# fevzibabaoglu/adaptive-edge-aware-jpeg

Measured on AMD Instinct MI355X. Metric: megapixels/sec encode (Canny+quadtree+DCT+quant), 4K batch, higher is better.
Workload: dtype f32

## Files before the change

adaptive_edge_aware_jpeg_amd/csrc/canny.hip:

```cpp
#include "aej_common.h"
#include "aej_launch.h"
#include <stdlib.h>

namespace aej {

__device__ __forceinline__ int reflect101(int i, int n)
{
    if (n == 1) return 0;
    while (i < 0 || i >= n) {
        if (i < 0) i = -i;
        if (i >= n) i = 2 * (n - 1) - i;
    }
    return i;
}

__device__ __forceinline__ int cdiv(int a, int b) { return (a + b - 1) / b; }

__device__ __forceinline__ long long xcd_remap(long long id, long long n)
{
    const long long q = n / 8, r = n % 8, xcd = id % 8, k = id / 8;
    return (xcd < r ? xcd * (q + 1) : r * (q + 1) + (xcd - r) * q) + k;
}

__device__ __forceinline__ bool locate_tile(const Geom &g, int TW, int TH, int t, int &layer, int &tx, int &ty, int &ntx, int &nty, int &tbase)
{
    tbase = 0;
    for (int l = 0; l < g.nl; l++) {
        ntx = cdiv(g.w[l], TW); nty = cdiv(g.h[l], TH);
        int n = ntx * nty;
        if (t < n) { layer = l; ty = t / ntx; tx = t - ty * ntx; return true; }
        t -= n; tbase += n;
    }
    return false;
}

static long long tiles_per_image(const Geom &g, int TW, int TH)
{
    long long n = 0;
    for (int l = 0; l < g.nl; l++) n += (long long)((g.w[l] + TW - 1) / TW) * ((g.h[l] + TH - 1) / TH);
    return n;
}
long long hyst_tiles_per_image(const Geom &g) { return tiles_per_image(g, kHystTile, kHystTile); }
int hyst_ring_slots(const Geom &g)
{
    const long long t2 = 2 * hyst_tiles_per_image(g) * g.B;
    int p = 1;
    while (2LL * p <= t2) p *= 2;
    return p;
}

__global__ __launch_bounds__(256) void k_clahe_pad_hist(Geom g, const unsigned char *__restrict__ u8, int *__restrict__ tile_hist)
{
    const int l = blockIdx.y, b = blockIdx.z;
    const int w = g.w[l], h = g.h[l];
    if ((w % 4) == 0 && (h % 4) == 0) return;
    const int wp = g.ctw[l] * 4, hp = g.cth[l] * 4;
    const int nright = (wp - w) * hp;
    const int nbottom = w * (hp - h);
    const unsigned char *src = u8 + (long long)b * g.pstride + g.poff[l];
    int *hist = tile_hist + ((long long)b * 3 + l) * 16 * 256;
    for (int i = blockIdx.x * 256 + threadIdx.x; i < nright + nbottom; i += gridDim.x * 256) {
        int x, y;
        if (i < nright) { y = i / (wp - w); x = w + (i - y * (wp - w)); }
        else { int k = i - nright; y = h + k / w; x = k % w; }
        int v = src[(long long)reflect101(y, h) * w + reflect101(x, w)];
        atomicAdd(&hist[((y / g.cth[l]) * 4 + (x / g.ctw[l])) * 256 + v], 1);
    }
}

__global__ __launch_bounds__(256) void k_clahe_lut(Geom g, const int *__restrict__ tile_hist, unsigned char *__restrict__ lut, double clip_limit)
{
    __shared__ int s[256];
    __shared__ int s_red[4];
    const int tile = blockIdx.x, l = blockIdx.y, b = blockIdx.z, tid = threadIdx.x;
    const long long base = (((long long)b * 3 + l) * 16 + tile) * 256;
    const int area = g.ctw[l] * g.cth[l];
    const float lutScale = 255.0f / (float)area;
    int clip = 0x7fffffff;
    if (clip_limit > 0.0) { clip = (int)(clip_limit * (double)area / 256.0); if (clip < 1) clip = 1; }
    int hv = tile_hist[base + tid];
    int excess = hv > clip ? hv - clip : 0;
    if (hv > clip) hv = clip;
    int v = excess;
    for (int o = 32; o > 0; o >>= 1) v += __shfl_down(v, o);
    if ((tid & 63) == 0) s_red[tid >> 6] = v;
    __syncthreads();
    const int clipped = s_red[0] + s_red[1] + s_red[2] + s_red[3];
    const int batch = clipped / 256;
    int resid = clipped - batch * 256;
    hv += batch;
    if (resid != 0) {
        int step = 256 / resid;
        if (step < 1) step = 1;
        if (tid % step == 0 && tid / step < resid) hv++;
    }
    s[tid] = hv;
    __syncthreads();
    for (int o = 1; o < 256; o <<= 1) {
        int t = tid >= o ? s[tid - o] : 0;
        __syncthreads();
        s[tid] += t;
        __syncthreads();
    }
    float f = (float)s[tid] * lutScale;
    int r = __float2int_rn(f);
    lut[base + tid] = (unsigned char)(r < 0 ? 0 : r > 255 ? 255 : r);
}

constexpr int kBT = 256;
constexpr int kBTW = 128, kBTH = 32;
constexpr int kBAW = kBTW + 8;
constexpr int kBAW4 = kBAW / 4;
constexpr int kBAH = kBTH + 6;
constexpr int kBGH = kBTH + 4;
constexpr int kBGW = kBAW + 4;
constexpr int kBGW2 = kBGW / 2;
static_assert(kBGW % 4 == 0, "Gaussian rows keep 8-byte alignment");
constexpr int kBStripMax = 15;
constexpr int kASlots = kBT / kBAW4;
constexpr int kAIter = (kBAH + kASlots - 1) / kASlots;
constexpr int kBRows = (kBGH + kASlots - 1) / kASlots;
static_assert(kASlots * kBRows >= kBGH && kASlots * kAIter >= kBAH, "thread -> row mapping must cover the tile");
constexpr float kTwo24 = 16777216.0f, kTwo22 = 4194304.0f;
constexpr int kHistCopies = 6;
constexpr int kHistStride = 257;

struct __attribute__((aligned(16))) BlurLds {
    int colq[kBAW];
    float colXa[kBAW], colXa1[kBAW];
    int colT1[kBAW], colT2[kBAW];
    int rowq[kBAH];
    float rowYa[kBAH], rowYa1[kBAH];
    int rowT1[kBAH], rowT2[kBAH];
    int cls[8];
    int pkey[2];
    float cw[3][512];
    unsigned int hist[kHistCopies * kHistStride];
    float4 P[2][256];
    unsigned int A[kBAH * kBAW4];
    unsigned int G[kBGH * kBGW2];
};
static_assert(3 * sizeof(BlurLds) <= 160 * 1024, "three workgroups per CU");

__device__ __forceinline__ int half_diff(unsigned a, int ah, unsigned b, int bh)
{
    int d;
    if (ah == 0 && bh == 0) asm("v_sub_u32_sdwa %0, %1, %2 dst_sel:DWORD dst_unused:UNUSED_PAD src0_sel:WORD_0 src1_sel:WORD_0" : "=v"(d) : "v"(b), "v"(a));
    else if (ah == 0)       asm("v_sub_u32_sdwa %0, %1, %2 dst_sel:DWORD dst_unused:UNUSED_PAD src0_sel:WORD_1 src1_sel:WORD_0" : "=v"(d) : "v"(b), "v"(a));
    else if (bh == 0)       asm("v_sub_u32_sdwa %0, %1, %2 dst_sel:DWORD dst_unused:UNUSED_PAD src0_sel:WORD_0 src1_sel:WORD_1" : "=v"(d) : "v"(b), "v"(a));
    else                    asm("v_sub_u32_sdwa %0, %1, %2 dst_sel:DWORD dst_unused:UNUSED_PAD src0_sel:WORD_1 src1_sel:WORD_1" : "=v"(d) : "v"(b), "v"(a));
    return d;
}

template <int T>
__device__ __forceinline__ float pair_w(const BlurLds &L, unsigned a, int ah, unsigned b, int bh)
{
    return *reinterpret_cast<const float *>(reinterpret_cast<const char *>(L.cw[T]) + 1024 + half_diff(a, ah, b, bh));
}

__device__ __forceinline__ float tap_fma(unsigned p, int h, float wgt, float sum)
{
    float r;
    if (h) asm("v_fma_mix_f32 %0, %1, %2, %3 op_sel:[1,0,0] op_sel_hi:[1,0,0]" : "=v"(r) : "v"(p), "v"(wgt), "v"(sum));
    else   asm("v_fma_mix_f32 %0, %1, %2, %3 op_sel_hi:[1,0,0]" : "=v"(r) : "v"(p), "v"(wgt), "v"(sum));
    return r;
}
__device__ __forceinline__ float tap_first(unsigned p, int h, float wgt)
{
    float r;
    if (h) asm("v_fma_mix_f32 %0, %1, %2, 0 op_sel:[1,0,0] op_sel_hi:[1,0,0]" : "=v"(r) : "v"(p), "v"(wgt));
    else   asm("v_fma_mix_f32 %0, %1, %2, 0 op_sel_hi:[1,0,0]" : "=v"(r) : "v"(p), "v"(wgt));
    return r;
}

__device__ __forceinline__ float clahe_blend(float l11, float l12, float l21, float l22, float xa, float xa1, float ya, float ya1)
{
    float pa = l11 * xa1, pb = l12 * xa, pc = l21 * xa1, pd = l22 * xa;
    float top = pa + pb, bot = pc + pd;
    float t1 = top * ya1, t2 = bot * ya;
    return t1 + t2;
}

__device__ __forceinline__ void blur_prefetch(const unsigned char *src, int w, int h, int x0, int y0, bool aligned, unsigned int (&raw)[kAIter])
{
    const int t = threadIdx.x;
    const int col = t % kBAW4, slot = t / kBAW4;
    if (slot >= kASlots) return;
#pragma unroll
    for (int k = 0; k < kAIter; k++) {
        const int j = slot + kASlots * k;
        if (j < kBAH) {
            if (aligned) {
                raw[k] = *reinterpret_cast<const unsigned int *>(src + (long long)(y0 - 3 + j) * w + (x0 - 4) + 4 * col);
            } else {
                const unsigned char *row = src + (long long)reflect101(y0 - 3 + j, h) * w;
                unsigned int v = 0;
#pragma unroll
                for (int q = 0; q < 4; q++) v |= (unsigned int)row[reflect101(x0 - 4 + 4 * col + q, w)] << (8 * q);
                raw[k] = v;
            }
        }
    }
}

__device__ __forceinline__ bool locate_blur_strip(const Geom &g, int strip, int t, int &layer, int &sx, int &ty)
{
    for (int l = 0; l < g.nl; l++) {
        int ntx = cdiv(g.w[l], kBTW), nty = cdiv(g.h[l], kBTH), nsx = cdiv(ntx, strip);
        int n = nsx * nty;
        if (t < n) { layer = l; ty = t / nsx; sx = t - ty * nsx; return true; }
        t -= n;
    }
    return false;
}


template <bool DUMP>
__global__ __launch_bounds__(kBT) __attribute__((amdgpu_waves_per_eu(3, 3))) void k_clahe_blur(Geom g, CannyBuffers cb, int strip)
{
    __shared__ BlurLds L;
    const int tid = threadIdx.x;
    const long long wg = xcd_remap(blockIdx.x, gridDim.x);
    const int strips = gridDim.x / g.B;
    const int b = (int)(wg / strips);
    int l, sx, ty;
    if (!locate_blur_strip(g, strip, (int)(wg - (long long)b * strips), l, sx, ty)) return;
    const int w = g.w[l], h = g.h[l];
    const int ntx = cdiv(w, kBTW);
    const int y0 = ty * kBTH;
    const int tx_begin = sx * strip, tx_end = min(ntx, tx_begin + strip);
    const long long pbase = (long long)b * g.pstride + g.poff[l];
    const unsigned char *src = cb.u8a + pbase;
    const unsigned char *glut = cb.lut + ((long long)b * 3 + l) * 4096;

    auto is_aligned = [&](int tx) {
        int x0 = tx * kBTW;
        return x0 >= 4 && y0 >= 3 && x0 + kBTW + 4 <= w && y0 + kBTH + 3 <= h && (w % 4) == 0;
    };
    unsigned int raw[kAIter];
    blur_prefetch(src, w, h, tx_begin * kBTW, y0, is_aligned(tx_begin), raw);

    static_assert(512 % kBT == 0, "weight table set-up assumes whole rounds");
#pragma unroll
    for (int i = tid; i < 512; i += kBT) {
        const int d = i - 256;
        const float cwv = i == 0 ? 0.f : cb.color_w[d < 0 ? -d : d];
        L.cw[0][i] = (cb.space_w[5] * cwv) * kTwo24;
        L.cw[1][i] = (cb.space_w[1] * cwv) * kTwo24;
        L.cw[2][i] = (cb.space_w[0] * cwv) * kTwo24;
    }
    for (int i = tid; i < kHistCopies * kHistStride; i += kBT) L.hist[i] = 0;
    if (tid < 2) L.pkey[tid] = -1;
    if (tid < kBAH) {
        const int j = tid;
        const int gy = reflect101(y0 - 3 + j, h);
        const float inv_th = 1.0f / (float)g.cth[l];
        float tyf = (float)gy * inv_th - 0.5f;
        int ty1 = (int)floorf(tyf), ty2 = ty1 + 1;
        float ya = tyf - (float)ty1;
        L.rowYa[j] = ya; L.rowYa1[j] = 1.0f - ya;
        if (ty1 < 0) ty1 = 0;
        if (ty2 > 3) ty2 = 3;
        L.rowT1[j] = ty1; L.rowT2[j] = ty2;
    }
    __syncthreads();
    {
        bool rchg = false;
        if (tid < kBAH) {
            const int j = tid;
            const int key = (L.rowT1[j] << 2) | L.rowT2[j], key0 = (L.rowT1[0] << 2) | L.rowT2[0];
            rchg = j > 0 && key != ((L.rowT1[j - 1] << 2) | L.rowT2[j - 1]);
            if (rchg) L.cls[3] = key;
            if (j == 0) L.cls[2] = key;
            L.rowq[j] = key != key0 ? (int)sizeof(L.P[0]) : 0;
        }
        const int n = __syncthreads_count(rchg);
        if (tid == 0) L.cls[5] = n;
    }
    unsigned char *dst = cb.u8b + pbase;

    for (int tx = tx_begin; tx < tx_end; tx++) {
        const int x0 = tx * kBTW;
        const bool full = x0 + kBTW <= w && y0 + kBTH <= h && (w % 4) == 0;
        if (tid == 0) L.cls[4] = 0;
        if (tid < kBAW) {
            const int gx = reflect101(x0 - 4 + tid, w);
            const float inv_tw = 1.0f / (float)g.ctw[l];
            float txf = (float)gx * inv_tw - 0.5f;
            int tx1 = (int)floorf(txf), tx2 = tx1 + 1;
            float xa = txf - (float)tx1;
            L.colXa[tid] = xa; L.colXa1[tid] = 1.0f - xa;
            if (tx1 < 0) tx1 = 0;
            if (tx2 > 3) tx2 = 3;
            L.colT1[tid] = tx1; L.colT2[tid] = tx2;
        }
        __syncthreads();
        if (tid < kBAW) {
            const int key = (L.colT1[tid] << 2) | L.colT2[tid], key0 = (L.colT1[0] << 2) | L.colT2[0];
            const bool chg = tid > 0 && key != ((L.colT1[tid - 1] << 2) | L.colT2[tid - 1]);
            if (chg) { atomicAdd(&L.cls[4], 1); L.cls[1] = key; }
            if (tid == 0) { L.cls[0] = key; }
            L.colq[tid] = key != key0 ? (int)sizeof(L.P[0]) : 0;
        }
        __syncthreads();
        const int nchg_c = L.cls[4], nchg_r = L.cls[5];
        const bool fast = nchg_c + nchg_r <= 1;
        if (fast) {
            const int key_s0 = (L.cls[0] << 4) | L.cls[2];
            const int key_s1 = (L.cls[nchg_c] << 4) | L.cls[2 + nchg_r];
            const bool need1 = nchg_c + nchg_r == 1;
            const bool build0 = L.pkey[0] != key_s0, build1 = need1 && L.pkey[1] != key_s1;
            if (build0 || build1) {
                for (int e = tid; e < 512; e += kBT) {
                    const int v = e & 255, slot = e >> 8;
                    const int key = slot ? key_s1 : key_s0;
                    if (slot ? build1 : build0) {
                        const int ckey = key >> 4, rkey = key & 15;
                        const int tx1 = ckey >> 2, tx2 = ckey & 3, ty1 = rkey >> 2, ty2 = rkey & 3;
                        L.P[slot][v] = make_float4((float)glut[(ty1 * 4 + tx1) * 256 + v], (float)glut[(ty1 * 4 + tx2) * 256 + v],
                                                   (float)glut[(ty2 * 4 + tx1) * 256 + v], (float)glut[(ty2 * 4 + tx2) * 256 + v]);
                    }
                }
                __syncthreads();
                if (tid < 2 && (tid ? build1 : build0)) L.pkey[tid] = tid ? key_s1 : key_s0;
            }
        }
        int tq = tid;
        asm volatile("" : "+v"(tq));
        const int acol = tq % kBAW4, aslot = tq / kBAW4;
        if (aslot < kASlots) {
            const float4 xa = reinterpret_cast<const float4 *>(L.colXa)[acol], xa1 = reinterpret_cast<const float4 *>(L.colXa1)[acol];
            if (fast) {
                const int4 cq = reinterpret_cast<const int4 *>(L.colq)[acol];
                const char *Pb = reinterpret_cast<const char *>(&L.P[0][0]);
#pragma unroll
                for (int k = 0; k < kAIter; k++) {
                    const int j = aslot + kASlots * k;
                    if (j < kBAH) {
                        const unsigned int rv = raw[k];
                        const int rq = L.rowq[j];
                        const float ya = L.rowYa[j], ya1 = L.rowYa1[j];
                        const float4 f0 = *reinterpret_cast<const float4 *>(Pb + ((rv & 0xffu) * 16u + (unsigned)(cq.x + rq)));
                        const float4 f1 = *reinterpret_cast<const float4 *>(Pb + (((rv >> 8) & 0xffu) * 16u + (unsigned)(cq.y + rq)));
                        const float4 f2 = *reinterpret_cast<const float4 *>(Pb + (((rv >> 16) & 0xffu) * 16u + (unsigned)(cq.z + rq)));
                        const float4 f3 = *reinterpret_cast<const float4 *>(Pb + ((rv >> 24) * 16u + (unsigned)(cq.w + rq)));
                        unsigned int o = __builtin_amdgcn_cvt_pk_u8_f32(clahe_blend(f0.x, f0.y, f0.z, f0.w, xa.x, xa1.x, ya, ya1), 0, 0u);
                        o = __builtin_amdgcn_cvt_pk_u8_f32(clahe_blend(f1.x, f1.y, f1.z, f1.w, xa.y, xa1.y, ya, ya1), 1, o);
                        o = __builtin_amdgcn_cvt_pk_u8_f32(clahe_blend(f2.x, f2.y, f2.z, f2.w, xa.z, xa1.z, ya, ya1), 2, o);
                        o = __builtin_amdgcn_cvt_pk_u8_f32(clahe_blend(f3.x, f3.y, f3.z, f3.w, xa.w, xa1.w, ya, ya1), 3, o);
                        L.A[j * kBAW4 + acol] = o;
                    }
                }
            } else {
                const int4 t1 = reinterpret_cast<const int4 *>(L.colT1)[acol], t2 = reinterpret_cast<const int4 *>(L.colT2)[acol];
                const int ct1[4] = { t1.x, t1.y, t1.z, t1.w }, ct2[4] = { t2.x, t2.y, t2.z, t2.w };
                const float cxa[4] = { xa.x, xa.y, xa.z, xa.w }, cxa1[4] = { xa1.x, xa1.y, xa1.z, xa1.w };
                for (int k = 0; k < kAIter; k++) {
                    const int j = aslot + kASlots * k;
                    if (j < kBAH) {
                        const unsigned int rv = raw[k];
                        const int r1 = L.rowT1[j] * 1024, r2 = L.rowT2[j] * 1024;
                        const float ya = L.rowYa[j], ya1 = L.rowYa1[j];
                        unsigned int o = 0;
#pragma unroll
                        for (int q = 0; q < 4; q++) {
                            const int v = (rv >> (8 * q)) & 0xff;
                            const float res = clahe_blend((float)glut[r1 + ct1[q] * 256 + v], (float)glut[r1 + ct2[q] * 256 + v],
                                                          (float)glut[r2 + ct1[q] * 256 + v], (float)glut[r2 + ct2[q] * 256 + v], cxa[q], cxa1[q], ya, ya1);
                            o = __builtin_amdgcn_cvt_pk_u8_f32(res, q, o);
                        }
                        L.A[j * kBAW4 + acol] = o;
                    }
                }
            }
        }
        if (tx + 1 < tx_end) blur_prefetch(src, w, h, (tx + 1) * kBTW, y0, is_aligned(tx + 1), raw);
        __syncthreads();
        if (DUMP && cb.dump_clahe)
            for (int idx = tid; idx < kBTH * kBTW; idx += kBT) {
                int j = idx / kBTW, i = idx - j * kBTW;
                if (x0 + i < w && y0 + j < h)
                    cb.dump_clahe[pbase + (long long)(y0 + j) * w + x0 + i] = reinterpret_cast<const unsigned char *>(L.A)[(j + 3) * kBAW + i + 4];
            }
        if (aslot < kASlots) {
            const int i4 = acol;
            const int il = i4 > 0 ? i4 - 1 : 0, ir = i4 < kBAW4 - 1 ? i4 + 1 : kBAW4 - 1;
            const int jg0 = aslot * kBRows;
            unsigned int he1 = 0, he2 = 0, ho1 = 0, ho2 = 0;
#pragma unroll
            for (int rr = 0; rr < kBRows + 2; rr++) {
                const int ja = jg0 + rr;
                if (ja < kBAH) {
                    const unsigned int *row = L.A + ja * kBAW4;
                    const unsigned int m = row[i4], lf = row[il], rt = row[ir];
                    const unsigned int LE = __builtin_amdgcn_perm(m, lf, 0x0C050C03u);
                    const unsigned int Am = m & 0x00FF00FFu;
                    const unsigned int Bm = __builtin_amdgcn_perm(m, m, 0x0C030C01u);
                    const unsigned int RO = __builtin_amdgcn_perm(rt, m, 0x0C040C02u);
                    const unsigned int he = LE + 2u * Am + Bm, ho = Am + 2u * Bm + RO;
                    if (rr >= 2 && ja - 2 < kBGH) {
                        const unsigned int ve = he2 + 2u * he1 + he + 0x00080008u;
                        const unsigned int vo = ho2 + 2u * ho1 + ho + 0x00080008u;
                        const unsigned int e4 = (ve >> 2) & 0x03FC03FCu;
                        const unsigned int o4 = (vo >> 2) & 0x03FC03FCu;
                        unsigned int *gp = &L.G[(ja - 2) * kBGW2 + 2 * i4 + 1];
                        gp[0] = __builtin_amdgcn_perm(o4, e4, 0x05040100u);
                        gp[1] = __builtin_amdgcn_perm(o4, e4, 0x07060302u);
                    }
                    he2 = he1; he1 = he; ho2 = ho1; ho1 = ho;
                }
            }
        }
        __syncthreads();
        if (DUMP && cb.dump_gauss)
            for (int idx = tid; idx < kBTH * kBTW; idx += kBT) {
                int j = idx / kBTW, i = idx - j * kBTW;
                if (x0 + i < w && y0 + j < h)
                    cb.dump_gauss[pbase + (long long)(y0 + j) * w + x0 + i] = (unsigned char)(reinterpret_cast<const unsigned short *>(L.G)[(j + 2) * kBGW + i + 6] >> 2);
            }
        int tc = tid;
        asm volatile("" : "+v"(tc));
        const int c4 = tc & 31;
        unsigned int *hcopy = L.hist + (tc % kHistCopies) * kHistStride;
        static_assert(kBTH == 4 * (kBT / 32), "one group of four rows per 32 threads");
        unsigned int W[8][4];
        {
            typedef unsigned int u32x2 __attribute__((ext_vector_type(2)));
            u32x2 m[16];
            const unsigned int base = (unsigned int)(size_t)(L.G + 4 * (tc >> 5) * kBGW2 + 2 * c4 + 2);
            constexpr int RS = kBGW2 * 4;
            static_assert(7 * RS + 8 < 65536 && (RS % 8) == 0, "DS offset field, alignment");
            asm volatile("ds_read_b64 %0, %16\n\tds_read_b64 %1, %16 offset:8\n\t"
                         "ds_read_b64 %2, %16 offset:%c17\n\tds_read_b64 %3, %16 offset:%c18\n\t"
                         "ds_read_b64 %4, %16 offset:%c19\n\tds_read_b64 %5, %16 offset:%c20\n\t"
                         "ds_read_b64 %6, %16 offset:%c21\n\tds_read_b64 %7, %16 offset:%c22\n\t"
                         "ds_read_b64 %8, %16 offset:%c23\n\tds_read_b64 %9, %16 offset:%c24\n\t"
                         "ds_read_b64 %10, %16 offset:%c25\n\tds_read_b64 %11, %16 offset:%c26\n\t"
                         "ds_read_b64 %12, %16 offset:%c27\n\tds_read_b64 %13, %16 offset:%c28\n\t"
                         "ds_read_b64 %14, %16 offset:%c29\n\tds_read_b64 %15, %16 offset:%c30\n\t"
                         "s_waitcnt lgkmcnt(0)"
                         : "=&v"(m[0]), "=&v"(m[1]), "=&v"(m[2]), "=&v"(m[3]), "=&v"(m[4]), "=&v"(m[5]), "=&v"(m[6]), "=&v"(m[7]), "=&v"(m[8]),
                           "=&v"(m[9]), "=&v"(m[10]), "=&v"(m[11]), "=&v"(m[12]), "=&v"(m[13]), "=&v"(m[14]), "=&v"(m[15])
                         : "v"(base), "i"(RS), "i"(RS + 8), "i"(2 * RS), "i"(2 * RS + 8), "i"(3 * RS), "i"(3 * RS + 8), "i"(4 * RS), "i"(4 * RS + 8),
                           "i"(5 * RS), "i"(5 * RS + 8), "i"(6 * RS), "i"(6 * RS + 8), "i"(7 * RS), "i"(7 * RS + 8)
                         : "memory");
#pragma unroll
            for (int wr = 0; wr < 8; wr++) {
                W[wr][0] = m[2 * wr].x; W[wr][1] = m[2 * wr].y; W[wr][2] = m[2 * wr + 1].x; W[wr][3] = m[2 * wr + 1].y;
            }
        }
        float two24 = kTwo24;
        asm volatile("" : "+s"(two24));
        auto PW0 = [&](int ar, int ac, int br, int bc) { return pair_w<0>(L, W[ar][ac >> 1], ac & 1, W[br][bc >> 1], bc & 1); };
        auto PW1 = [&](int ar, int ac, int br, int bc) { return pair_w<1>(L, W[ar][ac >> 1], ac & 1, W[br][bc >> 1], bc & 1); };
        auto PW2 = [&](int ar, int ac, int br, int bc) { return pair_w<2>(L, W[ar][ac >> 1], ac & 1, W[br][bc >> 1], bc & 1); };
        float cV1[4], cV2a[4], cV2b[4], cD1[4], cD2[4];
#pragma unroll
        for (int it = 0; it < 2; it++) {
            const int ro = 2 * it;
            const int yy = 4 * (tc >> 5) + ro;
            float sums[8], wsums[8];
            float V1m[4], D1m[5], D2m[5];
#pragma unroll
            for (int c = 0; c < 4; c++) V1m[c] = PW0(ro + 2, c + 2, ro + 3, c + 2);
#pragma unroll
            for (int i = 0; i < 5; i++) {
                D1m[i] = PW1(ro + 2, 1 + i, ro + 3, 2 + i);
                D2m[i] = PW1(ro + 2, 2 + i, ro + 3, 1 + i);
            }
#pragma unroll
            for (int r = 0; r < 2; r++) {
                float H1[5], H2[6], V1o[4], V2a[4], V2b[4], D1o[4], D2o[4];
#pragma unroll
                for (int i = 0; i < 5; i++) H1[i] = PW0(ro + r + 2, 1 + i, ro + r + 2, 2 + i);
#pragma unroll
                for (int i = 0; i < 6; i++) H2[i] = PW2(ro + r + 2, i, ro + r + 2, i + 2);
#pragma unroll
                for (int c = 0; c < 4; c++) {
                    V2a[c] = it == 1 ? (r == 0 ? cV2a[c] : cV2b[c]) : PW2(ro + r, c + 2, ro + r + 2, c + 2);
                    V2b[c] = PW2(ro + r + 2, c + 2, ro + r + 4, c + 2);
                    if (r == 0) {
                        V1o[c] = it == 1 ? cV1[c] : PW0(ro + 1, c + 2, ro + 2, c + 2);
                        D1o[c] = it == 1 && c >= 1 ? cD1[c - 1] : PW1(ro + 1, 1 + c, ro + 2, 2 + c);
                        D2o[c] = it == 1 && c <= 2 ? cD2[c + 1] : PW1(ro + 1, 3 + c, ro + 2, 2 + c);
                    } else {
                        V1o[c] = PW0(ro + 3, c + 2, ro + 4, c + 2);
                        D1o[c] = PW1(ro + 3, 2 + c, ro + 4, 3 + c);
                        D2o[c] = PW1(ro + 3, 2 + c, ro + 4, 1 + c);
                    }
                }
                if (it == 0) {
#pragma unroll
                    for (int c = 0; c < 4; c++) {
                        if (r == 0) cV2a[c] = V2b[c];
                        else { cV2b[c] = V2b[c]; cV1[c] = V1o[c]; cD1[c] = D1o[c]; cD2[c] = D2o[c]; }
                    }
                }
#pragma unroll
                for (int c = 0; c < 4; c++) {
                    auto tap = [&](float &sum, float &wsum, int wr, int wc, float wgt) {
                        wsum = wsum + wgt;
                        sum = tap_fma(W[ro + wr][wc >> 1], wc & 1, wgt, sum);
                    };
                    float wsum = V2a[c];
                    float sum = tap_first(W[ro + r][(c + 2) >> 1], (c + 2) & 1, V2a[c]);
                    tap(sum, wsum, r + 1, c + 1, r == 0 ? D1o[c] : D1m[c]);
                    tap(sum, wsum, r + 1, c + 2, r == 0 ? V1o[c] : V1m[c]);
                    tap(sum, wsum, r + 1, c + 3, r == 0 ? D2o[c] : D2m[c + 1]);
                    tap(sum, wsum, r + 2, c, H2[c]);
                    tap(sum, wsum, r + 2, c + 1, H1[c]);
                    tap(sum, wsum, r + 2, c + 2, two24);
                    tap(sum, wsum, r + 2, c + 3, H1[c + 1]);
                    tap(sum, wsum, r + 2, c + 4, H2[c + 2]);
                    tap(sum, wsum, r + 3, c + 1, r == 0 ? D2m[c] : D2o[c]);
                    tap(sum, wsum, r + 3, c + 2, r == 0 ? V1m[c] : V1o[c]);
                    tap(sum, wsum, r + 3, c + 3, r == 0 ? D1m[c + 1] : D1o[c]);
                    tap(sum, wsum, r + 4, c + 2, V2b[c]);
                    sums[r * 4 + c] = sum; wsums[r * 4 + c] = wsum;
                }
                __builtin_amdgcn_sched_barrier(0);
            }
            float z[8];
#pragma unroll
            for (int r = 0; r < 2; r++) {
                bool amb = false;
#pragma unroll
                for (int c = 0; c < 4; c++) {
                    const int q = r * 4 + c;
                    z[q] = (sums[q] * __builtin_amdgcn_rcpf(wsums[q])) * kTwo22;
                    amb = amb || (__builtin_fabsf(__builtin_amdgcn_fractf(z[q]) - 0.5f) < 1.220703125e-4f);
                }
                if (__any(amb)) {
#pragma unroll
                    for (int c = 0; c < 4; c++) z[r * 4 + c] = (sums[r * 4 + c] / wsums[r * 4 + c]) * kTwo22;
                }
            }
#pragma unroll
            for (int r = 0; r < 2; r++) {
                unsigned int packed = 0;
#pragma unroll
                for (int c = 0; c < 4; c++) packed = __builtin_amdgcn_cvt_pk_u8_f32(z[r * 4 + c], c, packed);
                const int y = y0 + yy + r;
                if (full) {
                    *reinterpret_cast<unsigned int *>(dst + (long long)y * w + x0 + 4 * c4) = packed;
                    if (packed == (packed & 0xffu) * 0x01010101u) {
                        atomicAdd(&hcopy[packed & 0xffu], 4u);
                    } else {
#pragma unroll
                        for (int c = 0; c < 4; c++) atomicAdd(&hcopy[(packed >> (8 * c)) & 0xffu], 1u);
                    }
                } else if (y < h) {
#pragma unroll
                    for (int c = 0; c < 4; c++)
                        if (x0 + 4 * c4 + c < w) {
                            dst[(long long)y * w + x0 + 4 * c4 + c] = (unsigned char)(packed >> (8 * c));
                            atomicAdd(&hcopy[(packed >> (8 * c)) & 0xffu], 1u);
                        }
                }
            }
        }
    }
    __syncthreads();
    if (tid < 256) {
        unsigned int c = 0;
#pragma unroll
        for (int k = 0; k < kHistCopies; k++) c += L.hist[k * kHistStride + tid];
        if (c) atomicAdd(&cb.blur_hist[((long long)b * 3 + l) * 256 + tid], (int)c);
    }
}

__device__ __forceinline__ double pct_from(const int *cum , const int *val_at , long long n, double q, int tid,
                                           int *s_a, int *s_b)
{
    (void)val_at;
    double virt = (double)(n - 1) * (q / 100.0);
    long long lo = (long long)floor(virt);
    long long hi = lo + 1;
    if (hi > n - 1) hi = n - 1;
    int prev = tid == 0 ? 0 : cum[tid - 1];
    int cur = cum[tid];
    if ((long long)cur > lo && (long long)prev <= lo) *s_a = tid;
    if ((long long)cur > hi && (long long)prev <= hi) *s_b = tid;
    __syncthreads();
    double t = virt - (double)lo;
    double a = (double)*s_a, bb = (double)*s_b;
    double diff = bb - a;
    double r = a + diff * t;
    if (t >= 0.5) r = bb - diff * (1.0 - t);
    __syncthreads();
    return r;
}

__global__ __launch_bounds__(256) void k_thresholds(Geom g, const int *__restrict__ blur_hist, int *__restrict__ thr, double low_q, double high_q, int l2)
{
    __shared__ int cum[256];
    __shared__ int s_a, s_b;
    const int l = blockIdx.x, b = blockIdx.y, tid = threadIdx.x;
    cum[tid] = blur_hist[((long long)b * 3 + l) * 256 + tid];
    __syncthreads();
    for (int o = 1; o < 256; o <<= 1) {
        int t = tid >= o ? cum[tid - o] : 0;
        __syncthreads();
        cum[tid] += t;
        __syncthreads();
    }
    long long n = (long long)g.w[l] * g.h[l];
    double lo = pct_from(cum, nullptr, n, low_q, tid, &s_a, &s_b);
    double hi = pct_from(cum, nullptr, n, high_q, tid, &s_a, &s_b);
    if (tid == 0) {
        if (lo > hi) { double t = lo; lo = hi; hi = t; }
        if (l2) {
            if (lo > 32767.0) lo = 32767.0;
            if (hi > 32767.0) hi = 32767.0;
            if (lo > 0) lo *= lo;
            if (hi > 0) hi *= hi;
        }
        thr[((long long)b * 3 + l) * 2 + 0] = (int)floor(lo);
        thr[((long long)b * 3 + l) * 2 + 1] = (int)floor(hi);
    }
}

constexpr int kStripMax = 8;

__device__ __forceinline__ bool locate_strip(const Geom &g, int strip, int t, int &layer, int &sx, int &ty)
{
    for (int l = 0; l < g.nl; l++) {
        int ntx = cdiv(g.w[l], kBlurTW), nty = cdiv(g.h[l], kBlurTH), nsx = cdiv(ntx, strip);
        int n = nsx * nty;
        if (t < n) { layer = l; ty = t / nsx; sx = t - ty * nsx; return true; }
        t -= n;
    }
    return false;
}

constexpr int kNW4 = (kBlurTW + 8) / 4;
constexpr int kNUH = kBlurTH + 4;
constexpr int kNMH = kBlurTH + 2;
constexpr int kNMW = kBlurTW + 8;
constexpr int kNRaw = (kNUH * kNW4 + 255) / 256;
constexpr int kS1Rows = 3;
static_assert((256 / kNW4) * kS1Rows >= kNMH, "stage-1 thread -> row mapping must cover the magnitude rows");

struct __attribute__((aligned(16))) NmsLds {
    int M[kNMH * kNMW];
    int G[kNMH * kNMW];
// ... 585 lines not shown
__global__ __launch_bounds__(256) void k_bits_to_edge(Geom g, const unsigned long long *__restrict__ strong, unsigned char *__restrict__ edge)
{
    const int l = blockIdx.y, b = blockIdx.z;
    const int w = g.w[l], h = g.h[l], wpr = g.wpr[l];
    const unsigned long long *sg = strong + (long long)b * g.bpstride + g.bpoff[l];
    unsigned char *out = edge + (long long)b * g.pstride + g.poff[l];
    const long long n = (long long)w * h;
    for (long long i = (long long)blockIdx.x * 256 + threadIdx.x; i < n; i += (long long)gridDim.x * 256) {
        int y = (int)(i / w), x = (int)(i - (long long)y * w);
        out[i] = (unsigned char)((sg[bp_index(y, x >> 6, wpr)] >> (x & 63)) & 1ull);
    }
}

__global__ __launch_bounds__(256) void k_bits_to_map(Geom g, const unsigned long long *__restrict__ weak, const unsigned long long *__restrict__ strong,
                                                     unsigned char *__restrict__ map)
{
    const int l = blockIdx.y, b = blockIdx.z;
    const int w = g.w[l], h = g.h[l], wpr = g.wpr[l];
    const unsigned long long *sg = strong + (long long)b * g.bpstride + g.bpoff[l];
    const unsigned long long *wk = weak + (long long)b * g.bpstride + g.bpoff[l];
    unsigned char *out = map + (long long)b * g.pstride + g.poff[l];
    const long long n = (long long)w * h;
    for (long long i = (long long)blockIdx.x * 256 + threadIdx.x; i < n; i += (long long)gridDim.x * 256) {
        int y = (int)(i / w), x = (int)(i - (long long)y * w);
        long long o = bp_index(y, x >> 6, wpr);
        int s = (int)((sg[o] >> (x & 63)) & 1ull), k = (int)((wk[o] >> (x & 63)) & 1ull);
        out[i] = (unsigned char)(s ? 2 : k ? 0 : 1);
    }
}

__global__ __launch_bounds__(256) void k_pack_edge_bits(Geom g, const unsigned char *__restrict__ edge, unsigned long long *__restrict__ bits)
{
    const int l = blockIdx.y, b = blockIdx.z;
    const int w = g.w[l], h = g.h[l], wpr = g.wpr[l];
    const unsigned char *src = edge + (long long)b * g.pstride + g.poff[l];
    unsigned long long *out = bits + (long long)b * g.bpstride + g.bpoff[l];
    const long long nwords = (long long)h * wpr;
    const int lane = threadIdx.x & 63;
    for (long long wd = (long long)blockIdx.x * 4 + (threadIdx.x >> 6); wd < nwords; wd += (long long)gridDim.x * 4) {
        int y = (int)(wd / wpr), xw = (int)(wd - (long long)y * wpr);
        int x = xw * 64 + lane;
        bool e = x < w && src[(long long)y * w + x] != 0;
        unsigned long long m = __ballot(e);
        if (lane == 0) out[bp_index(y, xw, wpr)] = m;
    }
}

__global__ __launch_bounds__(256) void k_zero16(uint4 *__restrict__ p, long long n16)
{
    for (long long i = (long long)blockIdx.x * 256 + threadIdx.x; i < n16; i += (long long)gridDim.x * 256) p[i] = make_uint4(0u, 0u, 0u, 0u);
}

void launch_zero(hipStream_t st, void *p, size_t bytes)
{
    const long long n16 = (long long)(bytes / 16);
    if (n16 <= 0) return;
    long long blocks = (n16 + 255) / 256;
    if (blocks > 4096) blocks = 4096;
    hipLaunchKernelGGL(k_zero16, dim3((unsigned)blocks), dim3(256), 0, st, reinterpret_cast<uint4 *>(p), n16);
}

void launch_clahe_pad_hist(hipStream_t st, const Geom &g, const CannyBuffers &cb)
{
    bool need = false;
    int maxpad = 0;
    for (int l = 0; l < g.nl; l++)
        if ((g.w[l] % 4) || (g.h[l] % 4)) {
            need = true;
            int wp = g.ctw[l] * 4, hp = g.cth[l] * 4;
            int n = (wp - g.w[l]) * hp + g.w[l] * (hp - g.h[l]);
            if (n > maxpad) maxpad = n;
        }
    if (!need) return;
    int bx = (maxpad + 255) / 256;
    if (bx > 1024) bx = 1024;
    hipLaunchKernelGGL(k_clahe_pad_hist, dim3(bx, g.nl, g.B), dim3(256), 0, st, g, cb.u8a, cb.tile_hist);
}

void launch_clahe_lut(hipStream_t st, const Geom &g, const CannyBuffers &cb)
{
    hipLaunchKernelGGL(k_clahe_lut, dim3(16, g.nl, g.B), dim3(256), 0, st, g, cb.tile_hist, cb.lut, cb.clip_limit);
}

static long long strips_per_image(const Geom &g, int TW, int TH, int strip)
{
    long long t = 0;
    for (int l = 0; l < g.nl; l++) {
        int ntx = (g.w[l] + TW - 1) / TW, nty = (g.h[l] + TH - 1) / TH;
        t += (long long)((ntx + strip - 1) / strip) * nty;
    }
    return t;
}
static int pick_strip(const Geom &g, int TW, int TH, int strip_max, long long want_workgroups)
{
    int strip = strip_max;
    while (strip > 1 && strips_per_image(g, TW, TH, strip) * g.B < want_workgroups) strip = (strip + 1) >> 1;
    return strip;
}

void launch_clahe_blur(hipStream_t st, const Geom &g, const CannyBuffers &cb)
{
    int best = 8, best_waste = 1 << 30;
    for (int s = 5; s <= kBStripMax; s++) {
        int waste = 0;
        for (int l = 0; l < g.nl; l++) {
            const int ntx = (g.w[l] + kBTW - 1) / kBTW;
            waste += (ntx + s - 1) / s * s - ntx;
        }
        if (waste <= best_waste) { best_waste = waste; best = s; }
    }
    const int strip = pick_strip(g, kBTW, kBTH, best, 1024);
    if (cb.dump_clahe || cb.dump_gauss)
        hipLaunchKernelGGL(k_clahe_blur<true>, dim3((unsigned)(strips_per_image(g, kBTW, kBTH, strip) * g.B)), dim3(kBT), 0, st, g, cb, strip);
    else
        hipLaunchKernelGGL(k_clahe_blur<false>, dim3((unsigned)(strips_per_image(g, kBTW, kBTH, strip) * g.B)), dim3(kBT), 0, st, g, cb, strip);
}

void launch_thresholds(hipStream_t st, const Geom &g, const CannyBuffers &cb)
{
    hipLaunchKernelGGL(k_thresholds, dim3(g.nl, g.B), dim3(256), 0, st, g, cb.blur_hist, cb.thr, cb.low_q, cb.high_q, cb.l2);
}

void launch_sobel_nms(hipStream_t st, const Geom &g, const CannyBuffers &cb, const Tuning &tn)
{
    bool reg_ok = !tn.sobel_lds;
    for (int l = 0; l < g.nl; l++) reg_ok = reg_ok && (g.w[l] % 4) == 0 && g.w[l] >= 4;
    if (reg_ok) {
        const long long t = hyst_tiles_per_image(g), total = t * g.B;
        const dim3 rgrid((unsigned)((total + 3) / 4));
        const int xcd = tn.sobel_xcd;
        if (cb.l2) hipLaunchKernelGGL(k_sobel_nms_reg<true>, rgrid, dim3(256), 0, st, g, cb, t, total, xcd);
        else hipLaunchKernelGGL(k_sobel_nms_reg<false>, rgrid, dim3(256), 0, st, g, cb, t, total, xcd);
        return;
    }
    const int strip = pick_strip(g, kBlurTW, kBlurTH, kStripMax, 2048);
    const dim3 grid((unsigned)(strips_per_image(g, kBlurTW, kBlurTH, strip) * g.B));
    if (cb.l2) hipLaunchKernelGGL(k_sobel_nms<true>, grid, dim3(256), 0, st, g, cb, strip);
    else hipLaunchKernelGGL(k_sobel_nms<false>, grid, dim3(256), 0, st, g, cb, strip);
}

constexpr int kHystDrainWgs = 64;

int hyst_bulk_launches(const Geom &g)
{
    const long long total = hyst_tiles_per_image(g) * g.B;
    return total > 32768 ? 2 : total > 8192 ? 1 : 0;
}
void launch_hysteresis(hipStream_t st, const Geom &g, const CannyBuffers &cb)
{
    const long long t = hyst_tiles_per_image(g), total = t * g.B;
    if (total <= 0) return;
    const int nbulk = hyst_bulk_launches(g), ring_mask = hyst_ring_slots(g) - 1;
    long long blocks = (total + 3) / 4;
    if (blocks > 16384) blocks = 16384;
    if (nbulk == 0) hipLaunchKernelGGL(k_hyst_pass0<true>, dim3((unsigned)blocks), dim3(256), 0, st, g, cb, t, total, ring_mask);
    else hipLaunchKernelGGL(k_hyst_pass0<false>, dim3((unsigned)blocks), dim3(256), 0, st, g, cb, t, total, ring_mask);
    const unsigned bulk_blocks = (unsigned)((total + 4 * kBulkGroup - 1) / (4 * kBulkGroup));
    for (int k = 1; k <= nbulk; k++) {
        if (k == nbulk) hipLaunchKernelGGL(k_hyst_bulk<true>, dim3(bulk_blocks), dim3(256), 0, st, g, cb, t, total, k, ring_mask);
        else hipLaunchKernelGGL(k_hyst_bulk<false>, dim3(bulk_blocks), dim3(256), 0, st, g, cb, t, total, k, ring_mask);
    }
    long long drain = total <= 8192 ? (total + 15) / 16 : (total + 63) / 64;
    if (drain > kHystDrainWgs) drain = kHystDrainWgs;
    hipLaunchKernelGGL(k_hyst_drain, dim3((unsigned)drain), dim3(256), 0, st, g, cb, t, total, nbulk & 1, ring_mask);
}

static int expand_blocks(const Geom &g)
{
    long long n = 0;
    for (int l = 0; l < g.nl; l++) { long long m = (long long)g.w[l] * g.h[l]; if (m > n) n = m; }
    long long b = (n + 255) / 256;
    return (int)(b > 4096 ? 4096 : b < 1 ? 1 : b);
}

void launch_bits_to_edge(hipStream_t st, const Geom &g, const unsigned long long *strong, unsigned char *edge01)
{
    hipLaunchKernelGGL(k_bits_to_edge, dim3(expand_blocks(g), g.nl, g.B), dim3(256), 0, st, g, strong, edge01);
}

void launch_bits_to_map(hipStream_t st, const Geom &g, const unsigned long long *weak, const unsigned long long *strong, unsigned char *map)
{
    hipLaunchKernelGGL(k_bits_to_map, dim3(expand_blocks(g), g.nl, g.B), dim3(256), 0, st, g, weak, strong, map);
}

void launch_pack_edge_bits(hipStream_t st, const Geom &g, const unsigned char *edge, unsigned long long *bits)
{
    hipLaunchKernelGGL(k_pack_edge_bits, dim3(expand_blocks(g), g.nl, g.B), dim3(256), 0, st, g, edge, bits);
}

}
```

Measured before the change: 85240.

## Walk CLAHE+blur strips vertically and carry halo rows between tiles

Each workgroup of the fused CLAHE+Gaussian blur kernel now walks down a vertical strip of tiles instead of across a horizontal one. Overlapping CLAHE and Gaussian halo rows are carried in LDS from one tile to the next rather than reloaded and recomputed. Column interpolation classes are computed once per strip, row classes per tile via wave ballot/shuffle, and LUT plan keys live in registers. This trades some extra LDS copying and more complex row mapping for fewer global loads and less redundant halo arithmetic.

```diff
diff --git a/adaptive_edge_aware_jpeg_amd/csrc/canny.hip b/adaptive_edge_aware_jpeg_amd/csrc/canny.hip
--- a/adaptive_edge_aware_jpeg_amd/csrc/canny.hip
+++ b/adaptive_edge_aware_jpeg_amd/csrc/canny.hip
@@ -1,6 +1,7 @@
 #include "aej_common.h"
 #include "aej_launch.h"
 #include <stdlib.h>
+#include <type_traits>
 
 namespace aej {
 
@@ -116,11 +117,12 @@
 constexpr int kBGW = kBAW + 4;
 constexpr int kBGW2 = kBGW / 2;
 static_assert(kBGW % 4 == 0, "Gaussian rows keep 8-byte alignment");
-constexpr int kBStripMax = 15;
+constexpr int kBStripMax = 17;
 constexpr int kASlots = kBT / kBAW4;
 constexpr int kAIter = (kBAH + kASlots - 1) / kASlots;
-constexpr int kBRows = (kBGH + kASlots - 1) / kASlots;
-static_assert(kASlots * kBRows >= kBGH && kASlots * kAIter >= kBAH, "thread -> row mapping must cover the tile");
+constexpr int kANew = kBAH - kBTH;
+constexpr int kGCarry = kBGH - kBTH;
+static_assert(kANew - 2 == kGCarry, "the carried Gaussian rows end where the carried CLAHE rows start");
 constexpr float kTwo24 = 16777216.0f, kTwo22 = 4194304.0f;
 constexpr int kHistCopies = 6;
 constexpr int kHistStride = 257;
@@ -133,7 +135,6 @@
     float rowYa[kBAH], rowYa1[kBAH];
     int rowT1[kBAH], rowT2[kBAH];
     int cls[8];
-    int pkey[2];
     float cw[3][512];
     unsigned int hist[kHistCopies * kHistStride];
     float4 P[2][256];
@@ -181,14 +182,16 @@
     return t1 + t2;
 }
 
+template <bool FIRST>
 __device__ __forceinline__ void blur_prefetch(const unsigned char *src, int w, int h, int x0, int y0, bool aligned, unsigned int (&raw)[kAIter])
 {
+    constexpr int j0 = FIRST ? 0 : kANew, iters = (kBAH - j0 + kASlots - 1) / kASlots;
     const int t = threadIdx.x;
     const int col = t % kBAW4, slot = t / kBAW4;
     if (slot >= kASlots) return;
 #pragma unroll
-    for (int k = 0; k < kAIter; k++) {
-        const int j = slot + kASlots * k;
+    for (int k = 0; k < iters; k++) {
+        const int j = j0 + slot + kASlots * k;
         if (j < kBAH) {
             if (aligned) {
                 raw[k] = *reinterpret_cast<const unsigned int *>(src + (long long)(y0 - 3 + j) * w + (x0 - 4) + 4 * col);
@@ -203,15 +206,41 @@
     }
 }
 
-__device__ __forceinline__ bool locate_blur_strip(const Geom &g, int strip, int t, int &layer, int &sx, int &ty)
+__device__ __forceinline__ bool locate_blur_strip(const Geom &g, int strip, int t, int &layer, int &bx, int &sy)
 {
     for (int l = 0; l < g.nl; l++) {
-        int ntx = cdiv(g.w[l], kBTW), nty = cdiv(g.h[l], kBTH), nsx = cdiv(ntx, strip);
-        int n = nsx * nty;
-        if (t < n) { layer = l; ty = t / nsx; sx = t - ty * nsx; return true; }
+        int ntx = cdiv(g.w[l], kBTW), nty = cdiv(g.h[l], kBTH), nsy = cdiv(nty, strip);
+        int n = ntx * nsy;
+        if (t < n) { layer = l; sy = t / ntx; bx = t - sy * ntx; return true; }
         t -= n;
     }
     return false;
+}
+
+struct BlurRowClasses { int key0, key1, nchg; };
+__device__ __forceinline__ BlurRowClasses blur_rows(BlurLds &L, const Geom &g, int l, int h, int y0, int j0, int tid)
+{
+    const int lane = tid & 63, j = j0 + lane;
+    int key = 0;
+    if (j < kBAH) {
+        const int gy = reflect101(y0 - 3 + j, h);
+        const float inv_th = 1.0f / (float)g.cth[l];
+        float tyf = (float)gy * inv_th - 0.5f;
+        int ty1 = (int)floorf(tyf), ty2 = ty1 + 1;
+        float ya = tyf - (float)ty1;
+        if (ty1 < 0) ty1 = 0;
+        if (ty2 > 3) ty2 = 3;
+        key = (ty1 << 2) | ty2;
+        if (tid < 64) { L.rowYa[j] = ya; L.rowYa1[j] = 1.0f - ya; L.rowT1[j] = ty1; L.rowT2[j] = ty2; }
+    }
+    const int above = __shfl_up(key, 1);
+    const unsigned long long chg = __ballot(j < kBAH && lane > 0 && key != above);
+    BlurRowClasses rc;
+    rc.key0 = __builtin_amdgcn_readfirstlane(key);
+    rc.nchg = __popcll(chg);
+    rc.key1 = __builtin_amdgcn_readfirstlane(__shfl(key, chg ? __builtin_ctzll(chg) : 0));
+    if (tid < 64 && j < kBAH) L.rowq[j] = key != rc.key0 ? (int)sizeof(L.P[0]) : 0;
+    return rc;
 }
 
 
@@ -223,22 +252,20 @@
     const long long wg = xcd_remap(blockIdx.x, gridDim.x);
     const int strips = gridDim.x / g.B;
     const int b = (int)(wg / strips);
-    int l, sx, ty;
-    if (!locate_blur_strip(g, strip, (int)(wg - (long long)b * strips), l, sx, ty)) return;
+    int l, bx, sy;
+    if (!locate_blur_strip(g, strip, (int)(wg - (long long)b * strips), l, bx, sy)) return;
     const int w = g.w[l], h = g.h[l];
-    const int ntx = cdiv(w, kBTW);
-    const int y0 = ty * kBTH;
-    const int tx_begin = sx * strip, tx_end = min(ntx, tx_begin + strip);
+    const int nty = cdiv(h, kBTH);
+    const int x0 = bx * kBTW;
+    const int ty_begin = sy * strip, ty_end = min(nty, ty_begin + strip);
     const long long pbase = (long long)b * g.pstride + g.poff[l];
     const unsigned char *src = cb.u8a + pbase;
     const unsigned char *glut = cb.lut + ((long long)b * 3 + l) * 4096;
 
-    auto is_aligned = [&](int tx) {
-        int x0 = tx * kBTW;
-        return x0 >= 4 && y0 >= 3 && x0 + kBTW + 4 <= w && y0 + kBTH + 3 <= h && (w % 4) == 0;
-    };
+    const bool aligned_x = x0 >= 4 && x0 + kBTW + 4 <= w && (w % 4) == 0;
+    auto is_aligned = [&](int y0) { return aligned_x && y0 >= 3 && y0 + kBTH + 3 <= h; };
     unsigned int raw[kAIter];
-    blur_prefetch(src, w, h, tx_begin * kBTW, y0, is_aligned(tx_begin), raw);
+    blur_prefetch<true>(src, w, h, x0, ty_begin * kBTH, is_aligned(ty_begin * kBTH), raw);
 
     static_assert(512 % kBT == 0, "weight table set-up assumes whole rounds");
 #pragma unroll
@@ -250,92 +277,71 @@
         L.cw[2][i] = (cb.space_w[0] * cwv) * kTwo24;
     }
     for (int i = tid; i < kHistCopies * kHistStride; i += kBT) L.hist[i] = 0;
-    if (tid < 2) L.pkey[tid] = -1;
-    if (tid < kBAH) {
-        const int j = tid;
-        const int gy = reflect101(y0 - 3 + j, h);
-        const float inv_th = 1.0f / (float)g.cth[l];
-        float tyf = (float)gy * inv_th - 0.5f;
-        int ty1 = (int)floorf(tyf), ty2 = ty1 + 1;
-        float ya = tyf - (float)ty1;
-        L.rowYa[j] = ya; L.rowYa1[j] = 1.0f - ya;
-        if (ty1 < 0) ty1 = 0;
-        if (ty2 > 3) ty2 = 3;
-        L.rowT1[j] = ty1; L.rowT2[j] = ty2;
-    }
+    if (tid == 0) L.cls[4] = 0;
+    if (tid < kBAW) {
+        const int gx = reflect101(x0 - 4 + tid, w);
+        const float inv_tw = 1.0f / (float)g.ctw[l];
+        float txf = (float)gx * inv_tw - 0.5f;
+        int tx1 = (int)floorf(txf), tx2 = tx1 + 1;
+        float xa = txf - (float)tx1;
+        L.colXa[tid] = xa; L.colXa1[tid] = 1.0f - xa;
+        if (tx1 < 0) tx1 = 0;
+        if (tx2 > 3) tx2 = 3;
+        L.colT1[tid] = tx1; L.colT2[tid] = tx2;
+    }
+    BlurRowClasses rc = blur_rows(L, g, l, h, ty_begin * kBTH, 0, tid);
     __syncthreads();
     {
-        bool rchg = false;
-        if (tid < kBAH) {
-            const int j = tid;
-            const int key = (L.rowT1[j] << 2) | L.rowT2[j], key0 = (L.rowT1[0] << 2) | L.rowT2[0];
-            rchg = j > 0 && key != ((L.rowT1[j - 1] << 2) | L.rowT2[j - 1]);
-            if (rchg) L.cls[3] = key;
-            if (j == 0) L.cls[2] = key;
-            L.rowq[j] = key != key0 ? (int)sizeof(L.P[0]) : 0;
-        }
-        const int n = __syncthreads_count(rchg);
-        if (tid == 0) L.cls[5] = n;
-    }
-    unsigned char *dst = cb.u8b + pbase;
-
-    for (int tx = tx_begin; tx < tx_end; tx++) {
-        const int x0 = tx * kBTW;
-        const bool full = x0 + kBTW <= w && y0 + kBTH <= h && (w % 4) == 0;
-        if (tid == 0) L.cls[4] = 0;
-        if (tid < kBAW) {
-            const int gx = reflect101(x0 - 4 + tid, w);
-            const float inv_tw = 1.0f / (float)g.ctw[l];
-            float txf = (float)gx * inv_tw - 0.5f;
-            int tx1 = (int)floorf(txf), tx2 = tx1 + 1;
-            float xa = txf - (float)tx1;
-            L.colXa[tid] = xa; L.colXa1[tid] = 1.0f - xa;
-            if (tx1 < 0) tx1 = 0;
-            if (tx2 > 3) tx2 = 3;
-            L.colT1[tid] = tx1; L.colT2[tid] = tx2;
-        }
-        __syncthreads();
+        bool chg = false;
         if (tid < kBAW) {
             const int key = (L.colT1[tid] << 2) | L.colT2[tid], key0 = (L.colT1[0] << 2) | L.colT2[0];
-            const bool chg = tid > 0 && key != ((L.colT1[tid - 1] << 2) | L.colT2[tid - 1]);
+            chg = tid > 0 && key != ((L.colT1[tid - 1] << 2) | L.colT2[tid - 1]);
             if (chg) { atomicAdd(&L.cls[4], 1); L.cls[1] = key; }
             if (tid == 0) { L.cls[0] = key; }
             L.colq[tid] = key != key0 ? (int)sizeof(L.P[0]) : 0;
         }
         __syncthreads();
-        const int nchg_c = L.cls[4], nchg_r = L.cls[5];
-        const bool fast = nchg_c + nchg_r <= 1;
-        if (fast) {
-            const int key_s0 = (L.cls[0] << 4) | L.cls[2];
-            const int key_s1 = (L.cls[nchg_c] << 4) | L.cls[2 + nchg_r];
-            const bool need1 = nchg_c + nchg_r == 1;
-            const bool build0 = L.pkey[0] != key_s0, build1 = need1 && L.pkey[1] != key_s1;
-            if (build0 || build1) {
-                for (int e = tid; e < 512; e += kBT) {
-                    const int v = e & 255, slot = e >> 8;
-                    const int key = slot ? key_s1 : key_s0;
-                    if (slot ? build1 : build0) {
-                        const int ckey = key >> 4, rkey = key & 15;
-                        const int tx1 = ckey >> 2, tx2 = ckey & 3, ty1 = rkey >> 2, ty2 = rkey & 3;
-                        L.P[slot][v] = make_float4((float)glut[(ty1 * 4 + tx1) * 256 + v], (float)glut[(ty1 * 4 + tx2) * 256 + v],
-                                                   (float)glut[(ty2 * 4 + tx1) * 256 + v], (float)glut[(ty2 * 4 + tx2) * 256 + v]);
-                    }
-                }
-                __syncthreads();
-                if (tid < 2 && (tid ? build1 : build0)) L.pkey[tid] = tid ? key_s1 : key_s0;
-            }
-        }
-        int tq = tid;
-        asm volatile("" : "+v"(tq));
-        const int acol = tq % kBAW4, aslot = tq / kBAW4;
+    }
+    const int nchg_c = __builtin_amdgcn_readfirstlane(L.cls[4]);
+    const int ccls0 = __builtin_amdgcn_readfirstlane(L.cls[0]), ccls1 = __builtin_amdgcn_readfirstlane(L.cls[1]);
+    int pkey0 = -1, pkey1 = -1;
+    bool fast = false;
+    auto plan_luts = [&](const BlurRowClasses &r) {
+        fast = nchg_c + r.nchg <= 1;
+        if (!fast) return;
+        const int key_s0 = (ccls0 << 4) | r.key0;
+        const int key_s1 = ((nchg_c ? ccls1 : ccls0) << 4) | (r.nchg ? r.key1 : r.key0);
+        const bool need1 = nchg_c + r.nchg == 1;
+        const bool build0 = pkey0 != key_s0, build1 = need1 && pkey1 != key_s1;
+        if (build0 || build1) {
+            for (int e = tid; e < 512; e += kBT) {
+                const int v = e & 255, slot = e >> 8;
+                const int key = slot ? key_s1 : key_s0;
+                if (slot ? build1 : build0) {
+                    const int ckey = key >> 4, rkey = key & 15;
+                    const int tx1 = ckey >> 2, tx2 = ckey & 3, ty1 = rkey >> 2, ty2 = rkey & 3;
+                    L.P[slot][v] = make_float4((float)glut[(ty1 * 4 + tx1) * 256 + v], (float)glut[(ty1 * 4 + tx2) * 256 + v],
+                                               (float)glut[(ty2 * 4 + tx1) * 256 + v], (float)glut[(ty2 * 4 + tx2) * 256 + v]);
+                }
+            }
+        }
+        if (build0) pkey0 = key_s0;
+        if (build1) pkey1 = key_s1;
+    };
+    plan_luts(rc);
+    __syncthreads();
+    unsigned char *dst = cb.u8b + pbase;
+
+    auto stage_a = [&](auto first, int acol, int aslot) {
+        constexpr int j0 = decltype(first)::value ? 0 : kANew, iters = (kBAH - j0 + kASlots - 1) / kASlots;
         if (aslot < kASlots) {
             const float4 xa = reinterpret_cast<const float4 *>(L.colXa)[acol], xa1 = reinterpret_cast<const float4 *>(L.colXa1)[acol];
             if (fast) {
                 const int4 cq = reinterpret_cast<const int4 *>(L.colq)[acol];
                 const char *Pb = reinterpret_cast<const char *>(&L.P[0][0]);
 #pragma unroll
-                for (int k = 0; k < kAIter; k++) {
-                    const int j = aslot + kASlots * k;
+                for (int k = 0; k < iters; k++) {
+                    const int j = j0 + aslot + kASlots * k;
                     if (j < kBAH) {
                         const unsigned int rv = raw[k];
                         const int rq = L.rowq[j];
@@ -355,8 +361,8 @@
                 const int4 t1 = reinterpret_cast<const int4 *>(L.colT1)[acol], t2 = reinterpret_cast<const int4 *>(L.colT2)[acol];
                 const int ct1[4] = { t1.x, t1.y, t1.z, t1.w }, ct2[4] = { t2.x, t2.y, t2.z, t2.w };
                 const float cxa[4] = { xa.x, xa.y, xa.z, xa.w }, cxa1[4] = { xa1.x, xa1.y, xa1.z, xa1.w };
-                for (int k = 0; k < kAIter; k++) {
-                    const int j = aslot + kASlots * k;
+                for (int k = 0; k < iters; k++) {
+                    const int j = j0 + aslot + kASlots * k;
                     if (j < kBAH) {
                         const unsigned int rv = raw[k];
                         const int r1 = L.rowT1[j] * 1024, r2 = L.rowT2[j] * 1024;
@@ -374,23 +380,27 @@
                 }
             }
         }
-        if (tx + 1 < tx_end) blur_prefetch(src, w, h, (tx + 1) * kBTW, y0, is_aligned(tx + 1), raw);
-        __syncthreads();
-        if (DUMP && cb.dump_clahe)
-            for (int idx = tid; idx < kBTH * kBTW; idx += kBT) {
-                int j = idx / kBTW, i = idx - j * kBTW;
-                if (x0 + i < w && y0 + j < h)
-                    cb.dump_clahe[pbase + (long long)(y0 + j) * w + x0 + i] = reinterpret_cast<const unsigned char *>(L.A)[(j + 3) * kBAW + i + 4];
-            }
+    };
+    auto stage_b = [&](auto first, int acol, int aslot) {
+        constexpr int g0 = decltype(first)::value ? 0 : kGCarry, n = kBGH - g0, q = n / kASlots, r = n % kASlots;
         if (aslot < kASlots) {
             const int i4 = acol;
             const int il = i4 > 0 ? i4 - 1 : 0, ir = i4 < kBAW4 - 1 ? i4 + 1 : kBAW4 - 1;
-            const int jg0 = aslot * kBRows;
+            int cnt, jg0;
+            if constexpr (decltype(first)::value) {
+                cnt = q + (aslot < r ? 1 : 0);
+                jg0 = g0 + aslot * q + min(aslot, r);
+            } else {
+                static_assert(n == 32 && q == 4, "layout below is for 32 rows over 7 slots");
+                constexpr unsigned long long kStart = 14ull | 24ull << 6 | 9ull << 12 | 19ull << 18 | 4ull << 24 | 28ull << 30 | 32ull << 36;
+                cnt = q + (int)((0x1Du >> aslot) & 1u);
+                jg0 = (int)((kStart >> (6 * aslot)) & 63u);
+            }
             unsigned int he1 = 0, he2 = 0, ho1 = 0, ho2 = 0;
 #pragma unroll
-            for (int rr = 0; rr < kBRows + 2; rr++) {
+            for (int rr = 0; rr < q + 3; rr++) {
                 const int ja = jg0 + rr;
-                if (ja < kBAH) {
+                if (rr < cnt + 2) {
                     const unsigned int *row = L.A + ja * kBAW4;
                     const unsigned int m = row[i4], lf = row[il], rt = row[ir];
                     const unsigned int LE = __builtin_amdgcn_perm(m, lf, 0x0C050C03u);
@@ -398,7 +408,7 @@
                     const unsigned int Bm = __builtin_amdgcn_perm(m, m, 0x0C030C01u);
                     const unsigned int RO = __builtin_amdgcn_perm(rt, m, 0x0C040C02u);
                     const unsigned int he = LE + 2u * Am + Bm, ho = Am + 2u * Bm + RO;
-                    if (rr >= 2 && ja - 2 < kBGH) {
+                    if (rr >= 2) {
                         const unsigned int ve = he2 + 2u * he1 + he + 0x00080008u;
                         const unsigned int vo = ho2 + 2u * ho1 + ho + 0x00080008u;
                         const unsigned int e4 = (ve >> 2) & 0x03FC03FCu;
@@ -411,6 +421,31 @@
                 }
             }
         }
+    };
+
+    for (int ty = ty_begin; ty < ty_end; ty++) {
+        const int y0 = ty * kBTH;
+        const bool first = ty == ty_begin, next = ty + 1 < ty_end;
+        const bool full = x0 + kBTW <= w && y0 + kBTH <= h && (w % 4) == 0;
+        int tq = tid;
+        asm volatile("" : "+v"(tq));
+        const int acol = tq % kBAW4, aslot = tq / kBAW4;
+        if (first) {
+            stage_a(std::true_type(), acol, aslot);
+        } else {
+            for (int i = tq; i < kGCarry * kBGW2; i += kBT) L.G[i] = L.G[kBTH * kBGW2 + i];
+            stage_a(std::false_type(), acol, aslot);
+        }
+        if (next) blur_prefetch<false>(src, w, h, x0, y0 + kBTH, is_aligned(y0 + kBTH), raw);
+        __syncthreads();
+        if (DUMP && cb.dump_clahe)
+            for (int idx = tid; idx < kBTH * kBTW; idx += kBT) {
+                int j = idx / kBTW, i = idx - j * kBTW;
+                if (x0 + i < w && y0 + j < h)
+                    cb.dump_clahe[pbase + (long long)(y0 + j) * w + x0 + i] = reinterpret_cast<const unsigned char *>(L.A)[(j + 3) * kBAW + i + 4];
+            }
+        if (first) stage_b(std::true_type(), acol, aslot);
+        else stage_b(std::false_type(), acol, aslot);
         __syncthreads();
         if (DUMP && cb.dump_gauss)
             for (int idx = tid; idx < kBTH * kBTW; idx += kBT) {
@@ -418,6 +453,12 @@
                 if (x0 + i < w && y0 + j < h)
                     cb.dump_gauss[pbase + (long long)(y0 + j) * w + x0 + i] = (unsigned char)(reinterpret_cast<const unsigned short *>(L.G)[(j + 2) * kBGW + i + 6] >> 2);
             }
+        if (next) {
+            constexpr int a0 = DUMP ? 3 : 4;
+            for (int i = tq; i < (kANew - a0) * kBAW4; i += kBT) L.A[a0 * kBAW4 + i] = L.A[(a0 + kBTH) * kBAW4 + i];
+            rc = blur_rows(L, g, l, h, y0 + kBTH, kANew, tid);
+            plan_luts(rc);
+        }
         int tc = tid;
         asm volatile("" : "+v"(tc));
         const int c4 = tc & 31;
@@ -559,8 +600,8 @@
                 }
             }
         }
-    }
-    __syncthreads();
+        __syncthreads();
+    }
     if (tid < 256) {
         unsigned int c = 0;
 #pragma unroll
@@ -1312,19 +1353,19 @@
     hipLaunchKernelGGL(k_clahe_lut, dim3(16, g.nl, g.B), dim3(256), 0, st, g, cb.tile_hist, cb.lut, cb.clip_limit);
 }
 
-static long long strips_per_image(const Geom &g, int TW, int TH, int strip)
+static long long strips_per_image(const Geom &g, int TW, int TH, int strip, bool vertical = false)
 {
     long long t = 0;
     for (int l = 0; l < g.nl; l++) {
         int ntx = (g.w[l] + TW - 1) / TW, nty = (g.h[l] + TH - 1) / TH;
-        t += (long long)((ntx + strip - 1) / strip) * nty;
+        t += vertical ? (long long)ntx * ((nty + strip - 1) / strip) : (long long)((ntx + strip - 1) / strip) * nty;
     }
     return t;
 }
-static int pick_strip(const Geom &g, int TW, int TH, int strip_max, long long want_workgroups)
+static int pick_strip(const Geom &g, int TW, int TH, int strip_max, long long want_workgroups, bool vertical = false)
 {
     int strip = strip_max;
-    while (strip > 1 && strips_per_image(g, TW, TH, strip) * g.B < want_workgroups) strip = (strip + 1) >> 1;
+    while (strip > 1 && strips_per_image(g, TW, TH, strip, vertical) * g.B < want_workgroups) strip = (strip + 1) >> 1;
     return strip;
 }
 
@@ -1334,16 +1375,17 @@
     for (int s = 5; s <= kBStripMax; s++) {
         int waste = 0;
         for (int l = 0; l < g.nl; l++) {
-            const int ntx = (g.w[l] + kBTW - 1) / kBTW;
-            waste += (ntx + s - 1) / s * s - ntx;
+            const int nty = (g.h[l] + kBTH - 1) / kBTH;
+            waste += (nty + s - 1) / s * s - nty;
         }
         if (waste <= best_waste) { best_waste = waste; best = s; }
     }
-    const int strip = pick_strip(g, kBTW, kBTH, best, 1024);
+    const int strip = pick_strip(g, kBTW, kBTH, best, 1024, true);
+    const dim3 grid((unsigned)(strips_per_image(g, kBTW, kBTH, strip, true) * g.B));
     if (cb.dump_clahe || cb.dump_gauss)
-        hipLaunchKernelGGL(k_clahe_blur<true>, dim3((unsigned)(strips_per_image(g, kBTW, kBTH, strip) * g.B)), dim3(kBT), 0, st, g, cb, strip);
+        hipLaunchKernelGGL(k_clahe_blur<true>, grid, dim3(kBT), 0, st, g, cb, strip);
     else
-        hipLaunchKernelGGL(k_clahe_blur<false>, dim3((unsigned)(strips_per_image(g, kBTW, kBTH, strip) * g.B)), dim3(kBT), 0, st, g, cb, strip);
+        hipLaunchKernelGGL(k_clahe_blur<false>, grid, dim3(kBT), 0, st, g, cb, strip);
 }
 
 void launch_thresholds(hipStream_t st, const Geom &g, const CannyBuffers &cb)
```

Result: no change. 86260, median of 6 (+1.2%).
